# zhenghao2519/Beyond-Fixed-Forms

Measured on AMD Instinct MI355X. Metric: scenes/sec (2D->3D projection+refinement), 200k pts x 300 views, higher is better.
Workload: dtype f64

## Files before the change

### beyond_fixed_forms_amd/_lib.py

```python
from __future__ import annotations

import ctypes
import os
import time
from ctypes import c_double, c_float, c_int32, c_int64, c_void_p

import torch

_HERE = os.path.dirname(os.path.abspath(__file__))
LIB_PATH = os.environ.get("BFF_HIP_LIB") or os.path.join(_HERE, "lib", "libbff_hip.so")
CSRC_DIR = os.path.join(_HERE, "csrc")

_P, _I, _L, _D, _F = c_void_p, c_int32, c_int64, c_double, c_float

SIGNATURES = {
    "bff_rle_to_maskbits": [_P, _P, _P, _P, _I, _L, _I, _P, _P, _P],
    "bff_rle_to_labels": [_P, _P, _P, _P, _I, _L, _I, _P, _P, _P, _P],
    "bff_mask_row_directory": [_P, _P, _P, _I, _I, _I, _P, _P],
    "bff_project_views_lookup": [_P, _L, _L, _P, _P, _I, _P, _I, _I, _I, _P, _I, _I, _D, _P, _P, _P, _P, _P, _I, _P, _P, _P, _P, _P, _L, _L, _P, _P, _P, _P],
    "bff_project_views_cached": [_L, _I, _P, _I, _I, _P, _P, _P, _P, _P, _P, _P, _P, _I, _P, _P, _P, _P, _P, _L, _L, _P, _P, _P, _P],
    "bff_visibility_table": [_P, _L, _L, _P, _P, _I, _P, _I, _I, _I, _I, _I, _D, _P, _P, _P, _P, _L, _P, _I, _P],
    "bff_visibility_sorted": [_P, _P, _P, _L, _L, _I, _I, _I, _P, _P, _P, _P, _P, _P],
    "bff_project_views_runs": [_L, _I, _P, _I, _I, _P, _P, _P, _P, _P, _P, _P, _P, _I, _P, _P, _P, _P, _P, _L, _L, _P, _P, _P, _P],
    "bff_masks2d_count": [_P, _I, _L, _P, _P, _P],
    "bff_masks2d_runs": [_P, _I, _L, _P, _P, _P, _P],
    "bff_project_views": [_P, _L, _L, _P, _P, _I, _P, _P, _I, _I, _D, _P, _P, _P, _I, _P, _P, _P, _P, _P, _L, _L, _P, _P, _P, _P, _P],
    "bff_depth_tile_u16": [_P, _I, _I, _I, _P, _I, _P],
    "bff_project_views_u16": [_P, _L, _L, _P, _P, _I, _P, _I, _I, _I, _P, _I, _I, _D, _P, _P, _P, _I, _P, _P, _P, _P, _P, _L, _L, _P, _P, _P, _P, _P],
    "bff_point_tile_bounds": [_P, _L, _L, _P, _P],
    "bff_count_viewed": [_P, _L, _L, _P, _P, _I, _P, _I, _I, _I, _P, _I, _I, _D, _I, _P, _P, _P],
    "bff_render_depth_u16": [_P, _L, _L, _P, _P, _I, _I, _I, _I, _I, _I, _P, _P, _P, _P],
    "bff_render_splat_depth_u16": [_P, _L, _L, _P, _P, _I, _I, _I, _I, _I, _D, _I, _P, _P, _P, _P],
    "bff_point_labels": [_P, _I, _L, _L, _P, _P, _P],
    "bff_render_labels_u16": [_P, _L, _L, _P, _P, _P, _I, _I, _I, _I, _I, _D, _I, _P, _P, _P, _P, _P],
    "bff_label_runs_count": [_P, _I, _I, _I, _I, _I, _I, _P, _P, _P],
    "bff_label_runs_emit": [_P, _I, _I, _I, _I, _I, _I, _P, _L, _P, _P, _P, _P],
    "bff_render_mesh_depth_u16": [_P, _L, _L, _P, _L, _P, _P, _I, _I, _I, _I, _I, _I, _P, _P, _P],
    "bff_render_mesh_depth_clip_u16": [_P, _L, _L, _P, _L, _P, _P, _I, _I, _I, _I, _I, _D, _I, _P, _P, _P],
# ... 1020 lines not shown
```

### beyond_fixed_forms_amd/csrc/merge.hip

```cpp
#include <hip/hip_ext.h>

#include <cstdlib>

#include "rows.h"

static thread_local hipEvent_t g_merge_start = nullptr, g_merge_stop = nullptr;

namespace bff {

constexpr int kBins = 64;

__device__ __forceinline__ int64_t heavy_signature(uint64_t heavy)
{
    uint32_t key = 0;
#pragma unroll
    for (int s = 0; s < 5; ++s) {
        int b = 63;
        if (heavy) { b = __ffsll((unsigned long long)heavy) - 1; heavy &= heavy - 1; }
        key = (key << 6) | (uint32_t)b;
    }
    return (int64_t)key;
}

__global__ __launch_bounds__(256) void row_stats_kernel(const uint64_t *__restrict__ rows, int64_t nw, int mw,
                                                         int bin_words, int32_t *__restrict__ area,
                                                         int32_t *__restrict__ mean_word,
                                                         uint64_t *__restrict__ cmask, uint32_t *__restrict__ hist,
                                                         int64_t *__restrict__ signature, uint16_t *__restrict__ cpop)
{
    extern __shared__ uint64_t s_cm[];
    __shared__ int part[4];
    __shared__ unsigned long long psum[4];
    __shared__ uint32_t s_hist[kBins];
    const int r = blockIdx.x, tid = threadIdx.x;
    const uint64_t *row = rows + (int64_t)r * nw;
    for (int i = tid; i < mw; i += 256) s_cm[i] = 0;
    if (tid < kBins) s_hist[tid] = 0;
// ... 17 lines not shown
    __syncthreads();
    for (int i = tid; i < mw; i += 256) cmask[(int64_t)r * mw + i] = s_cm[i];
    if (cpop) {
        const int n_chunks = (int)((nw + kCW - 1) / kCW);
        for (int c = tid; c < mw * 64; c += 256) {
            int pc = 0;
            if (c < n_chunks)
#pragma unroll
                for (int k = 0; k < kCW; ++k) { const int64_t w = (int64_t)c * kCW + k; if (w < nw) pc += popc64(row[w]); }
            cpop[(int64_t)r * mw * 64 + c] = (uint16_t)pc;
        }
    }
    const int a_all = part[0] + part[1] + part[2] + part[3];
    if (tid < kBins) {
        hist[(int64_t)r * kBins + tid] = s_hist[tid];
        const uint64_t heavy = __ballot((uint64_t)s_hist[tid] * 100 >= (uint64_t)a_all * 15 && a_all > 0);
        if (tid == 0) signature[r] = heavy_signature(a_all ? heavy : 0);
    }
    if (tid == 0) {
        const int a = part[0] + part[1] + part[2] + part[3];
        const unsigned long long t = psum[0] + psum[1] + psum[2] + psum[3];
        area[r] = a;
        mean_word[r] = a ? (int32_t)(t / (unsigned long long)a) : 0x7fffffff;
    }
}

__global__ __launch_bounds__(256) void row_stats_sparse_kernel(const uint64_t *__restrict__ rows, int n_rows, int64_t nw,
                                                                int mw, int bin_words, int32_t *__restrict__ area,
                                                                int32_t *__restrict__ mean_word,
                                                                const uint64_t *__restrict__ cmask,
                                                                uint32_t *__restrict__ hist, int64_t *__restrict__ signature,
// ... 22 lines not shown
                    const int pc = popc64(v);
                    atomicAdd(&hs[(int)(w / bin_words)], (uint32_t)pc);
                    s += pc;
                    in_chunk += pc;
                    ws += (unsigned long long)pc * (unsigned long long)w;
                }
            }
            if (cpop) cpop[(int64_t)r * mw * 64 + i * 64 + lane] = (uint16_t)in_chunk;
        }
    }
#pragma unroll
    for (int d = 32; d > 0; d >>= 1) { s += __shfl_xor(s, d); ws += __shfl_xor(ws, d); }
    asm volatile("s_waitcnt lgkmcnt(0)" ::: "memory");
    const uint32_t hv = hs[lane];
    hist[(int64_t)r * kBins + lane] = hv;
    const uint64_t heavy = __ballot((uint64_t)hv * 100 >= (uint64_t)s * 15 && s > 0);
    if (lane == 0) {
        signature[r] = heavy_signature(s ? heavy : 0);
        area[r] = s;
        mean_word[r] = s ? (int32_t)(ws / (unsigned long long)s) : 0x7fffffff;
    }
}

__global__ __launch_bounds__(256) void tile_masks_kernel(const uint64_t *__restrict__ cmask,
                                                          const int32_t *__restrict__ order, int n, int mw,
                                                          uint64_t *__restrict__ tmask, const uint32_t *__restrict__ hist,
                                                          uint32_t *__restrict__ hist_sorted, int n_pos,
                                                          const int32_t *__restrict__ area,
                                                          uint32_t *__restrict__ tile_hmax, int32_t *__restrict__ tile_amin,
                                                          const int32_t *__restrict__ label_id,
                                                          int32_t *__restrict__ row_sorted, int32_t *__restrict__ area_sorted,
// ... 817 lines not shown
                             uint16_t *chunk_pop, void *stream)
{
    BFF_REQUIRE(n_rows >= 0 && nw >= 0, "bff_row_stats: bad sizes");
    if (n_rows == 0) return BFF_OK;
    BFF_REQUIRE(rows && area && mean_word && chunk_mask && hist && signature, "bff_row_stats: null pointer");
    const int n_chunks = (int)ceil_div(nw, kCW);
    BFF_LIMIT(n_chunks <= kMaxChunks, "bff_row_stats: more than %d chunks (N > %d points)", kMaxChunks, kMaxChunks * kCW * 64);
    const int mw = (int)ceil_div(n_chunks, 64);
    static_assert(kBins == kWave, "row_stats_sparse_kernel: one histogram bin per lane");
    if (chunk_mask_given) {
        if (chunk_pop) {
            hipError_t e = zero_async(chunk_pop, sizeof(uint16_t) * (size_t)n_rows * mw * 64, as_stream(stream));
            if (e != hipSuccess) return fail((int)e, "bff_row_stats: memset: %s", hipGetErrorString(e));
        }
        row_stats_sparse_kernel<<<(unsigned)ceil_div(n_rows, 4), 256, 0, as_stream(stream)>>>(
            rows, n_rows, nw, mw, (int)ceil_div(nw > 0 ? nw : 1, kBins), area, mean_word, chunk_mask, hist, signature, chunk_pop);
        return launched("bff_row_stats");
    }
    row_stats_kernel<<<n_rows, 256, mw * sizeof(uint64_t), as_stream(stream)>>>(
        rows, nw, mw, (int)ceil_div(nw > 0 ? nw : 1, kBins), area, mean_word, chunk_mask, hist, signature, chunk_pop);
    return launched("bff_row_stats");
}

extern "C" int bff_merge_adjacency(const uint64_t *rows, int32_t n_rows, int64_t nw, const int32_t *order,
                                   const uint64_t *chunk_mask, uint64_t *tile_mask, const uint32_t *hist,
                                   const int32_t *area,
                                   const int32_t *label_id, float iou_thres, uint64_t *adj, int32_t *inter,
                                   void *stream)
{
    BFF_REQUIRE(n_rows >= 0 && nw >= 0, "bff_merge_adjacency: bad sizes");
    if (n_rows == 0) return BFF_OK;
    BFF_REQUIRE(rows && area && label_id && adj, "bff_merge_adjacency: null pointer");
    BFF_REQUIRE((chunk_mask == nullptr) == (tile_mask == nullptr), "bff_merge_adjacency: chunk_mask and tile_mask go together");
    const int nt = (int)ceil_div(n_rows, kT);
    BFF_LIMIT((int64_t)nt * (nt + 1) / 2 < (1ll << 31), "bff_merge_adjacency: too many rows");
// ... 2 lines not shown
    const int mw = (int)ceil_div(n_chunks, 64);
    const bool sparse = chunk_mask && !(0.0f > iou_thres);
    if (sparse) tile_masks_kernel<<<nt, 256, 0, as_stream(stream)>>>(chunk_mask, order, n_rows, mw, tile_mask, nullptr, nullptr, 0, nullptr, nullptr, nullptr,
                                                                     nullptr, nullptr, nullptr, nullptr, nullptr);
    const int aw = nt;
    merge_adjacency_kernel<<<(unsigned)((int64_t)nt * (nt + 1) / 2), 256, 0, as_stream(stream)>>>(
        rows, n_rows, nw, order, sparse ? tile_mask : nullptr, mw, (sparse && !inter) ? hist : nullptr, area, label_id,
        iou_thres, adj, aw, inter, nt);
    return launched("bff_merge_adjacency");
}

extern "C" int32_t bff_merge_uses_chunk_bound(int64_t nw)
{
    static const int forced = [] { const char *e = getenv("BFF_CHUNK_BOUND"); return e ? atoi(e) : -1; }();
    if (forced >= 0) return forced != 0;
    return ceil_div(nw > 0 ? nw : 1, kBins) >= 4 * kCW;
}

struct MergeScratch {
    int64_t n_pos, total, cap2;
    int64_t hist_sorted, tile_hmax, tile_amin;
    int64_t row_sorted, area_sorted, label_sorted;
    int64_t counts, list1, list2;
    int64_t pass2, part2;
    int64_t arrive, partial;
    int64_t words;
};

static MergeScratch merge_scratch_layout(int64_t n)
{
    MergeScratch s;
// ... 117 lines not shown
```

### beyond_fixed_forms_amd/csrc/rows.h

```cpp
#pragma once

#include "common.h"

namespace bff {

constexpr int kT = 64;
constexpr int kKW = 32;
constexpr int kPitch = kT + 1;

__device__ __forceinline__ int uf_find(int32_t *parent, int x)
{
    int p = __hip_atomic_load(parent + x, __ATOMIC_RELAXED, __HIP_MEMORY_SCOPE_AGENT);
    while (p != x) {
        const int g = __hip_atomic_load(parent + p, __ATOMIC_RELAXED, __HIP_MEMORY_SCOPE_AGENT);
        if (g != p) __hip_atomic_store(parent + x, g, __ATOMIC_RELAXED, __HIP_MEMORY_SCOPE_AGENT);
        x = p;
        p = g;
    }
    return x;
}

__device__ __forceinline__ void uf_union(int32_t *parent, int a, int b)
{
    for (;;) {
// ... 20 lines not shown
```

### beyond_fixed_forms_amd/csrc/scene.hip

```cpp
#include "rows.h"

using namespace bff;

namespace {

__global__ void order_keys_kernel(const int64_t *__restrict__ sig, const int32_t *__restrict__ label_id, int n,
                                  int sig_bits, int64_t *__restrict__ keys)
{
    const int i = blockIdx.x * blockDim.x + threadIdx.x;
    if (i < n) keys[i] = ((int64_t)label_id[i] << sig_bits) | sig[i];
}

int bits_for(int n)
{
    int b = 1;
    while ((1 << b) < n && b < 31) ++b;
    return b;
}

}

#define BFF_TRY(call) do { const int rc_ = (call); if (rc_ != BFF_OK) return rc_; } while (0)

extern "C" int32_t bff_scene_header_words(int32_t s1_rows, int32_t cap)
// ... 66 lines not shown
        BFF_TRY(hand_over(ws->events[0], stream, hv));
    }
    const bool cached = lookup && sc->vis_mask && sc->vis_off && sc->vis_pix;
    const bool runs = cached && sc->vis_spix && sc->vis_spt && sc->vis_rowstart && bff_sweep_runs_ok(n) != 0;
    if (lookup && !runs) {
        BFF_REQUIRE(ws->mask_tab && ws->mask_dir, "bff_scene_project: no row directory buffers");
        BFF_TRY(bff_mask_row_directory(sc->run_start, sc->run_end, sc->mask_run_offs, n_rows, sc->height, sc->width,
                                       ws->mask_tab, ws->mask_dir, hv));
    } else if (!lookup) {
        BFF_TRY(bff_rle_to_labels(sc->run_start, sc->run_end, sc->mask_run_offs, sc->view_mask_offs, sc->n_mviews, hw,
                                  sc->word_bits, ws->labels, ws->maskbits, ws->segmap, hv));
    }
    const bool ratio = pr->filter_mode == 2;
    int32_t *const sweep_viewed = (ratio && !viewed_in) ? ws->viewed : nullptr;
    const int32_t *const viewed = ratio ? (viewed_in ? viewed_in : ws->viewed) : nullptr;
    if (runs)
        BFF_TRY(bff_project_views_runs(n, sc->n_frames, sc->depth_index, sc->height, sc->width, sc->vis_mask, sc->vis_spix,
                                       sc->vis_spt, sc->vis_rowstart, sc->run_start, sc->run_end, sc->mask_run_offs,
                                       sc->view_mask_offs, sc->word_bits, sc->frame_mask, sc->frame_rowbase, sc->frame_nmask,
                                       sc->frame_flags, ws->rows, n_rows, nw, ws->chunk_mask, ws->masked, sweep_viewed, hv));
    else if (cached)
        BFF_TRY(bff_project_views_cached(n, sc->n_frames, sc->depth_index, sc->height, sc->width, sc->vis_mask, sc->vis_off,
                                         sc->vis_pix, ws->mask_tab, ws->mask_dir, sc->run_start, sc->run_end,
                                         sc->view_mask_offs, sc->word_bits, sc->frame_mask, sc->frame_rowbase, sc->frame_nmask,
                                         sc->frame_flags, ws->rows, n_rows, nw, ws->chunk_mask, ws->masked, sweep_viewed, hv));
    else if (lookup)
        BFF_TRY(bff_project_views_lookup(sc->xyz, n, sc->n_pad, sc->inv_pose, sc->cam_intr, sc->n_frames,
                                         sc->depth_raw ? sc->depth_raw : (const void *)sc->depth, sc->depth_h, sc->depth_w,
                                         sc->depth_raw ? sc->depth_tiled : -1, sc->depth_index, sc->height, sc->width,
                                         pr->depth_thresh, ws->mask_tab, ws->mask_dir, sc->run_start, sc->run_end,
                                         sc->view_mask_offs, sc->word_bits, sc->frame_mask, sc->frame_rowbase, sc->frame_nmask,
                                         sc->frame_flags, ws->rows, n_rows, nw, ws->chunk_mask, ws->masked, sweep_viewed,
                                         sc->tile_bounds, hv));
    else if (sc->depth_raw)
        BFF_TRY(bff_project_views_u16(sc->xyz, n, sc->n_pad, sc->inv_pose, sc->cam_intr, sc->n_frames, sc->depth_raw,
                                      sc->depth_h, sc->depth_w, sc->depth_tiled, sc->depth_index, sc->height, sc->width, pr->depth_thresh,
// ... 23 lines not shown
        } else {
            BFF_TRY(bff_point_threshold_pairs(ws->masked, viewed, n, pr->filter_fraction,
                                              ws->pair_scratch, reinterpret_cast<float *>(hdr + BFF_HDR_THR),
                                              hdr + BFF_HDR_NUNIQUE, hdr + BFF_HDR_OVERFLOW, stream));
        }
        BFF_TRY(bff_ratio_keep(ws->masked, viewed, n, 0.0f,
                               reinterpret_cast<const float *>(hdr + BFF_HDR_THR), 1, nw, ws->keep, stream));
    } else {
        BFF_TRY(bff_ratio_keep(ws->masked, nullptr, n, 0.0f, nullptr, 0, nw, ws->keep, stream));
    }
    if (fork) {
        hipError_t ee = hipEventRecord(reinterpret_cast<hipEvent_t>(ws->aux_events[1]), as_stream(stream));
        if (ee != hipSuccess) return fail((int)ee, "bff_scene_project: aux stream: %s", hipGetErrorString(ee));
        stream = main_stream;
    }
    uint16_t *cpop = bff_merge_uses_chunk_bound(nw) ? ws->chunk_pop : nullptr;
    BFF_TRY(bff_row_stats(ws->rows, n_rows, nw, ws->area, ws->mean_word, ws->chunk_mask, 1, ws->hist, ws->sig, cpop, stream));
    {
        const int64_t *keys = ws->sig;
        int key_bits = BFF_SIGNATURE_BITS;
        if (sc->n_label_ids > 1) {
            key_bits += bits_for(sc->n_label_ids);
            order_keys_kernel<<<(unsigned)ceil_div(n_rows, 256), 256, 0, st>>>(ws->sig, sc->label_id, n_rows,
                                                                              BFF_SIGNATURE_BITS, ws->sig_keys);
            keys = ws->sig_keys;
        }
        size_t tb = ws->sort_temp_bytes;
        BFF_TRY(bff_argsort_i64(keys, ws->sig_sorted, ws->order, n_rows, key_bits, ws->sort_temp, &tb, stream));
    }
    BFF_TRY(merge_components_streams(ws->rows, n_rows, nw, ws->order, n_rows, ws->chunk_mask, ws->tile_mask, ws->hist,
                                     ws->merge_scratch, ws->area, sc->label_id, pr->iou_thres, ws->parent, 1, nullptr, nullptr,
                                     cpop, stream, hv, ws->events[2], ws->events[3]));
// ... 32 lines not shown
```

### beyond_fixed_forms_amd/csrc/sweep_runs.hip

```cpp
#include <algorithm>
#include <cstdlib>

#include <hip/hip_ext.h>
#include <rocprim/device/device_radix_sort.hpp>

#include "sweep.h"

namespace bff {


__global__ __launch_bounds__(kBlock) void vis_sort_keys_kernel(const uint64_t *__restrict__ mask, const uint32_t *__restrict__ off,
                                                               const uint32_t *__restrict__ pix, int64_t stride, int64_t n_pairs,
                                                               int W, uint32_t hw, uint32_t *__restrict__ keys,
                                                               uint32_t *__restrict__ pts)
{
    const int lane = threadIdx.x & 63;
    const int64_t w = (int64_t)blockIdx.x * (kBlock / kWave) + (threadIdx.x >> 6);
    const int slot = blockIdx.y;
    if (w >= stride) return;
    const uint64_t m = mask[slot * stride + w];
    if (!((m >> lane) & 1)) return;
    const int64_t at = (int64_t)off[slot * stride + w] + __popcll(m & ((1ull << lane) - 1));
    if (at >= n_pairs) return;
    const uint32_t p = pix[at];
// ... 15 lines not shown
    const int64_t t = (int64_t)blockIdx.x * kBlock + threadIdx.x;
    if (t >= (int64_t)n_slots * (H + 1)) return;
    const int s = (int)(t / (H + 1)), y = (int)(t - (int64_t)s * (H + 1));
    int64_t lo = min((int64_t)off[s * stride], n_pairs);
    int64_t hi = s + 1 < n_slots ? min((int64_t)off[(s + 1) * stride], n_pairs) : n_pairs;
    const uint32_t target = (uint32_t)y * (uint32_t)W;
    while (lo < hi) {
        const int64_t mid = lo + ((hi - lo) >> 1);
        if (spix[mid] < target) lo = mid + 1; else hi = mid;
    }
    rowstart[t] = (uint32_t)lo;
}

constexpr int kRunsDeal = 4;

__global__ __launch_bounds__(kBlock) void sweep_runs_fill_kernel(
    int n_frames, const int32_t *__restrict__ depth_index, int H, int W,
    const uint32_t *__restrict__ spix, const uint32_t *__restrict__ spt, const uint32_t *__restrict__ rowstart,
    const int32_t *__restrict__ run_start, const int32_t *__restrict__ run_end, const int32_t *__restrict__ mask_run_offs,
    const int32_t *__restrict__ view_mask_offs, const int32_t *__restrict__ frame_mask,
    const int32_t *__restrict__ frame_rowbase, const int32_t *__restrict__ frame_nmask,
    uint64_t *__restrict__ rows, int64_t nw, int n_chunks, uint64_t *__restrict__ chunk_mask, int mw)
{
    extern __shared__ uint64_t s_row[];
    const int f = blockIdx.x, m = blockIdx.y;
    const int mi = frame_mask[f];
    if (mi < 0 || m >= frame_nmask[f]) return;
    const int tid = threadIdx.x, lane = tid & 63, wave = tid >> 6;
    const int64_t row = (int64_t)frame_rowbase[f] + m;
    for (int i = tid; i < n_chunks * kCW; i += kBlock) s_row[i] = 0;
    __syncthreads();

    const int g = view_mask_offs[mi] + m;
    const int r0 = mask_run_offs[g], r1 = mask_run_offs[g + 1];
    const uint32_t *rs = rowstart + (int64_t)depth_index[f] * (H + 1);
    const int hw = H * W;
    uint32_t *bits = reinterpret_cast<uint32_t *>(s_row);
    for (int rb = r0 + wave * kWave; rb < r1; rb += kBlock) {
        const int r = rb + lane;
        uint32_t lo = 0, cnt = 0;
        if (r < r1) {
            const int start = max(run_start[r], 0), end = min(run_end[r], hw);
            if (start < end) {
                const int y = start / W, ye = (end - 1) / W;
                uint32_t lo1 = rs[y], hi1 = rs[y + 1], lo2 = rs[ye], hi2 = rs[ye + 1];
// ... 48 lines not shown
        for (int h = 0; h < kCW; h += kPPT) {
            uint64_t o = 0;
#pragma unroll
            for (int q = 0; q < kPPT; ++q) o |= v[h + q];
            if (o) {
                any = true;
#pragma unroll
                for (int q = 0; q < kPPT; ++q) {
                    const int64_t w = (int64_t)c * kCW + h + q;
                    if (w < nw) rows[row * nw + w] = v[h + q];
                }
            }
        }
        const uint64_t flags = __ballot(any);
        if (lane == 0 && flags) chunk_mask[row * mw + (c0 >> 6)] |= flags;
    }
}

constexpr int kCountBlock = 1024;
constexpr int kCountBatch = 4;
constexpr int kCountList = 4096;

__global__ __launch_bounds__(kCountBlock) void sweep_runs_count_kernel(const uint64_t *__restrict__ rows, int64_t n_rows, int64_t nw,
                                                                       const uint64_t *__restrict__ chunk_mask, int mw,
                                                                       int64_t n_points, int32_t *__restrict__ masked_count)
{
    __shared__ int s_cnt[kCW * kWave];
    __shared__ int s_list[kCountList];
    __shared__ int s_n;
    const int tid = threadIdx.x, lane = tid & 63, wave = tid >> 6;
    const int c = blockIdx.x;
    static_assert(kCountList == kCountBatch * kCountBlock, "a round lists what one batch of flag loads covers");
    for (int i = tid; i < kCW * kWave; i += kCountBlock) s_cnt[i] = 0;
    int cnt[8] = {};
    const int64_t word = (int64_t)c * kCW + (lane >> 3);
    const int shift = 8 * (lane & 7);
    const uint64_t *flag = chunk_mask + (c >> 6);
    for (int64_t r0 = 0; r0 < n_rows; r0 += kCountList) {
        if (tid == 0) s_n = 0;
        __syncthreads();
        bool set[kCountBatch];
#pragma unroll
        for (int k = 0; k < kCountBatch; ++k) {
            const int64_t r = r0 + k * kCountBlock + tid;
            set[k] = r < n_rows && ((flag[r * mw] >> (c & 63)) & 1);
        }
#pragma unroll
        for (int k = 0; k < kCountBatch; ++k)
            if (set[k]) s_list[atomicAdd(&s_n, 1)] = k * kCountBlock + tid;
        __syncthreads();
        const int n = s_n;
        for (int i0 = wave * kCountBatch; i0 < n; i0 += (kCountBlock / kWave) * kCountBatch) {
            uint64_t v[kCountBatch];
#pragma unroll
            for (int k = 0; k < kCountBatch; ++k)
                v[k] = (i0 + k < n && word < nw) ? rows[(r0 + s_list[i0 + k]) * nw + word] : 0;
#pragma unroll
            for (int k = 0; k < kCountBatch; ++k) {
                const uint32_t b = (uint32_t)(v[k] >> shift) & 0xffu;
#pragma unroll
// ... 7 lines not shown
        if (cnt[q]) atomicAdd(&s_cnt[8 * lane + q], cnt[q]);
    __syncthreads();
    for (int i = tid; i < kCW * kWave; i += kCountBlock) {
        const int64_t n = (int64_t)c * kCW * kWave + i;
        if (n < n_points && s_cnt[i]) masked_count[n] += s_cnt[i];
    }
}

constexpr int kViewedBatch = 4;

__global__ __launch_bounds__(kBlock) void sweep_runs_viewed_kernel(int n_frames, const int32_t *__restrict__ depth_index,
                                                                   const int32_t *__restrict__ frame_flags,
                                                                   const uint64_t *__restrict__ vis_mask, int64_t stride,
                                                                   int64_t nw, int64_t n_points, int32_t *__restrict__ viewed_count)
{
    const int lane = threadIdx.x & 63;
    const int64_t w = (int64_t)blockIdx.x * (kBlock / kWave) + (threadIdx.x >> 6);
    if (w >= nw) return;
    int cnt = 0;
    for (int f0 = 0; f0 < n_frames; f0 += kViewedBatch * kWave) {
        uint64_t m[kViewedBatch];
        int32_t slot[kViewedBatch], flags[kViewedBatch];
#pragma unroll
        for (int k = 0; k < kViewedBatch; ++k) {
            const int f = f0 + k * kWave + lane;
            slot[k] = f < n_frames ? depth_index[f] : 0;
            flags[k] = f < n_frames ? frame_flags[f] : 0;
        }
#pragma unroll
        for (int k = 0; k < kViewedBatch; ++k) m[k] = (flags[k] & 1) ? vis_mask[(int64_t)slot[k] * stride + w] : 0;
#pragma unroll
        for (int k = 0; k < kViewedBatch; ++k) {
            uint64_t live = __ballot(m[k] != 0);
            while (live) {
                const int l = __ffsll((unsigned long long)live) - 1;
                live &= live - 1;
                const uint32_t lo = (uint32_t)__builtin_amdgcn_readlane((int)(uint32_t)m[k], l);
                const uint32_t hi = (uint32_t)__builtin_amdgcn_readlane((int)(uint32_t)(m[k] >> 32), l);
                cnt += (int)(((((uint64_t)hi << 32) | lo) >> lane) & 1);
            }
        }
    }
    const int64_t n = w * kWave + lane;
    if (n < n_points && cnt) viewed_count[n] += cnt;
}

}

using namespace bff;

constexpr int64_t kRunsLdsMax = 64 * 1024;

static int64_t runs_row_bytes(int64_t n_points)
{
    return (int64_t)sizeof(uint64_t) * kCW * ceil_div(ceil_div(n_points, (int64_t)kWave), (int64_t)kCW);
}

extern "C" int32_t bff_sweep_runs_ok(int64_t n_points)
{
    const char *on = getenv("BFF_SWEEP_RUNS"), *cap = getenv("BFF_SWEEP_RUNS_LDS_BYTES");
    if (on && on[0] == '0' && on[1] == 0) return 0;
    int64_t bound = kRunsLdsMax;
    if (cap && *cap) bound = std::min<int64_t>(bound, std::max<int64_t>(0, atoll(cap)));
    return n_points > 0 && runs_row_bytes(n_points) <= bound;
}

extern "C" int bff_project_views_runs(int64_t n_points, int32_t n_frames, const int32_t *depth_index, int32_t height,
                                      int32_t width, const uint64_t *vis_mask, const uint32_t *vis_spix,
                                      const uint32_t *vis_spt, const uint32_t *vis_rowstart, const int32_t *run_start,
                                      const int32_t *run_end, const int32_t *mask_run_offs, const int32_t *view_mask_offs,
                                      int32_t word_bits, const int32_t *frame_mask, const int32_t *frame_rowbase,
                                      const int32_t *frame_nmask, const int32_t *frame_flags, uint64_t *rows, int64_t n_rows,
                                      int64_t nw, uint64_t *chunk_mask, int32_t *masked_count, int32_t *viewed_count,
                                      void *stream)
{
    if (n_points <= 0 || n_frames <= 0) return BFF_OK;
    BFF_REQUIRE(height > 0 && width > 0, "bff_project_views_runs: bad image size");
    BFF_LIMIT((int64_t)height * width < (1ll << 31), "bff_project_views_runs: image larger than 2^31 pixels");
    BFF_REQUIRE(vis_mask && vis_spix && vis_spt && vis_rowstart, "bff_project_views_runs: null table");
    BFF_REQUIRE(word_bits == 32 || word_bits == 64, "bff_project_views_runs: word_bits must be 32 or 64");
    BFF_REQUIRE(depth_index && frame_mask && frame_rowbase && frame_nmask && frame_flags && run_start && run_end &&
                mask_run_offs && view_mask_offs && rows && chunk_mask && n_rows >= 0, "bff_project_views_runs: null pointer");
    BFF_REQUIRE(nw == ceil_div(n_points, 64), "bff_project_views_runs: nw must be ceil(n_points/64)");
    const int64_t row_bytes = runs_row_bytes(n_points);
    BFF_LIMIT(row_bytes <= kRunsLdsMax, "bff_project_views_runs: an instance row exceeds 64 KB of LDS (bff_sweep_runs_ok)");
    hipStream_t st = as_stream(stream);
    const int n_chunks = (int)ceil_div(nw, kCW), mw = (int)ceil_div(n_chunks, 64);
    hipEvent_t ev0, ev1;
    take_sweep_events(&ev0, &ev1);
    const bool count = masked_count != nullptr && n_rows > 0, viewed = viewed_count != nullptr;
    hipExtLaunchKernelGGL(sweep_runs_fill_kernel, dim3((unsigned)n_frames, (unsigned)word_bits), dim3(kBlock),
        (unsigned)row_bytes, st, ev0, (count || viewed) ? nullptr : ev1, 0,
        n_frames, depth_index, height, width, vis_spix, vis_spt, vis_rowstart, run_start, run_end, mask_run_offs,
        view_mask_offs, frame_mask, frame_rowbase, frame_nmask, rows, nw, n_chunks, chunk_mask, mw);
    if (count)
        hipExtLaunchKernelGGL(sweep_runs_count_kernel, dim3((unsigned)n_chunks), dim3(kCountBlock), 0, st,
            nullptr, viewed ? nullptr : ev1, 0, rows, n_rows, nw, chunk_mask, mw, n_points, masked_count);
    if (viewed)
        hipExtLaunchKernelGGL(sweep_runs_viewed_kernel, dim3((unsigned)ceil_div(nw, kBlock / kWave)), dim3(kBlock), 0, st,
            nullptr, ev1, 0, n_frames, depth_index, frame_flags, vis_mask, bff_visibility_words(n_points), nw, n_points,
            viewed_count);
    return launched("bff_project_views_runs");
}

extern "C" int bff_visibility_sorted_bytes(int32_t n_slots, int32_t height, int64_t n_pixels, int64_t *bytes)
{
    BFF_REQUIRE(n_slots >= 0 && height >= 0 && n_pixels >= 0 && bytes, "bff_visibility_sorted_bytes: bad arguments");
    bytes[0] = (int64_t)sizeof(uint32_t) * n_pixels;
    bytes[1] = (int64_t)sizeof(uint32_t) * n_pixels;
    bytes[2] = (int64_t)sizeof(uint32_t) * n_slots * ((int64_t)height + 1);
    return BFF_OK;
}

extern "C" int bff_visibility_sorted(const uint64_t *vis_mask, const uint32_t *vis_off, const uint32_t *vis_pix,
                                     int64_t n_pixels, int64_t n_points, int32_t n_slots, int32_t height, int32_t width,
                                     uint32_t *vis_spix, uint32_t *vis_spt, uint32_t *vis_rowstart, void *temp,
                                     size_t *temp_bytes, void *stream)
// ... 38 lines not shown
```

### include/bff_hip.h

```cpp
#ifndef BFF_HIP_H
#define BFF_HIP_H

#include <stddef.h>
#include <stdint.h>

#ifdef __cplusplus
extern "C" {
#endif

#define BFF_OK 0
#define BFF_E_ARG (-1)
#define BFF_E_LIMIT (-2)

#define BFF_ABI_VERSION 16

int bff_abi_version(void);
const char *bff_last_error(void);
const char *bff_arch(void);

int bff_host_component_csr(const int32_t *comp, const uint8_t *has_self_loop, int32_t n, int32_t min_members,
                           int32_t *offs, int32_t *members, int32_t *sizes, int32_t *n_void);

int bff_rle_to_maskbits(const int32_t *run_start, const int32_t *run_end, const int32_t *mask_run_offs,
                        const int32_t *view_mask_offs, int32_t n_views, int64_t n_pixels, int32_t word_bits,
// ... 246 lines not shown
                             int32_t *masked_count, int32_t *viewed_count, void *stream);

int bff_visibility_sorted(const uint64_t *vis_mask, const uint32_t *vis_off, const uint32_t *vis_pix, int64_t n_pixels,
                          int64_t n_points, int32_t n_slots, int32_t height, int32_t width, uint32_t *vis_spix,
                          uint32_t *vis_spt, uint32_t *vis_rowstart, void *temp, size_t *temp_bytes, void *stream);
int bff_visibility_sorted_bytes(int32_t n_slots, int32_t height, int64_t n_pixels, int64_t *bytes);

int32_t bff_sweep_runs_ok(int64_t n_points);
int bff_project_views_runs(int64_t n_points, int32_t n_frames, const int32_t *depth_index, int32_t height, int32_t width,
                           const uint64_t *vis_mask, const uint32_t *vis_spix, const uint32_t *vis_spt,
                           const uint32_t *vis_rowstart, const int32_t *run_start, const int32_t *run_end,
                           const int32_t *mask_run_offs, const int32_t *view_mask_offs, int32_t word_bits,
                           const int32_t *frame_mask, const int32_t *frame_rowbase, const int32_t *frame_nmask,
                           const int32_t *frame_flags, uint64_t *rows, int64_t n_rows, int64_t nw, uint64_t *chunk_mask,
                           int32_t *masked_count, int32_t *viewed_count, void *stream);

typedef struct bff_scene {
    int64_t n_points, n_pad, nw;
    const double *xyz;
    const double *tile_bounds;
    const double *inv_pose;
    double cam_intr[9];
    const float *depth;
    const void *depth_raw;
    const int32_t *depth_index, *frame_mask, *frame_rowbase, *frame_nmask, *frame_flags;
    const int32_t *run_start, *run_end, *mask_run_offs, *view_mask_offs;
    const void *conf;
    const int32_t *label_id;
    const int32_t *unsort;
    const int32_t *perm;
// ... 151 lines not shown
```

Before: 1542.

## Fuse row statistics into runs sweep fill kernel and transpose chunk flags

Computes per-row area, mean word, histogram, heavy-bin signature and chunk popcounts inside the runs fill kernel while the row is still in LDS, so the separate row_stats pass over all rows is skipped on the runs path. The fill kernel also writes a transposed chunk-flag table into the mask_dir scratch, giving the count kernel contiguous flag reads. The viewed kernel is restructured so one block covers one word, with its waves splitting the frames and reducing through shared memory. In exchange the fill kernel gains LDS atomics and register pressure, and mask_dir is reused as scratch, which depends on the height/alignment check.

New measurement: 1508. -2.2%, worse.

```diff
diff --git a/beyond_fixed_forms_amd/_lib.py b/beyond_fixed_forms_amd/_lib.py
--- a/beyond_fixed_forms_amd/_lib.py
+++ b/beyond_fixed_forms_amd/_lib.py
@@ -22,6 +22,7 @@
     "bff_visibility_table": [_P, _L, _L, _P, _P, _I, _P, _I, _I, _I, _I, _I, _D, _P, _P, _P, _P, _L, _P, _I, _P],
     "bff_visibility_sorted": [_P, _P, _P, _L, _L, _I, _I, _I, _P, _P, _P, _P, _P, _P],
     "bff_project_views_runs": [_L, _I, _P, _I, _I, _P, _P, _P, _P, _P, _P, _P, _P, _I, _P, _P, _P, _P, _P, _L, _L, _P, _P, _P, _P],
+    "bff_project_views_runs_stats": [_L, _I, _P, _I, _I, _P, _P, _P, _P, _P, _P, _P, _P, _I, _P, _P, _P, _P, _P, _L, _L, _P, _P, _P] + [_P] * 7,
     "bff_masks2d_count": [_P, _I, _L, _P, _P, _P],
     "bff_masks2d_runs": [_P, _I, _L, _P, _P, _P, _P],
     "bff_project_views": [_P, _L, _L, _P, _P, _I, _P, _P, _I, _I, _D, _P, _P, _P, _I, _P, _P, _P, _P, _P, _L, _L, _P, _P, _P, _P, _P],
diff --git a/beyond_fixed_forms_amd/csrc/merge.hip b/beyond_fixed_forms_amd/csrc/merge.hip
--- a/beyond_fixed_forms_amd/csrc/merge.hip
+++ b/beyond_fixed_forms_amd/csrc/merge.hip
@@ -8,19 +8,6 @@
 
 namespace bff {
 
-constexpr int kBins = 64;
-
-__device__ __forceinline__ int64_t heavy_signature(uint64_t heavy)
-{
-    uint32_t key = 0;
-#pragma unroll
-    for (int s = 0; s < 5; ++s) {
-        int b = 63;
-        if (heavy) { b = __ffsll((unsigned long long)heavy) - 1; heavy &= heavy - 1; }
-        key = (key << 6) | (uint32_t)b;
-    }
-    return (int64_t)key;
-}
 
 __global__ __launch_bounds__(256) void row_stats_kernel(const uint64_t *__restrict__ rows, int64_t nw, int mw,
                                                          int bin_words, int32_t *__restrict__ area,
@@ -68,7 +55,7 @@
     const int a_all = part[0] + part[1] + part[2] + part[3];
     if (tid < kBins) {
         hist[(int64_t)r * kBins + tid] = s_hist[tid];
-        const uint64_t heavy = __ballot((uint64_t)s_hist[tid] * 100 >= (uint64_t)a_all * 15 && a_all > 0);
+        const uint64_t heavy = __ballot(heavy_bin(s_hist[tid], a_all));
         if (tid == 0) signature[r] = heavy_signature(a_all ? heavy : 0);
     }
     if (tid == 0) {
@@ -121,7 +108,7 @@
     asm volatile("s_waitcnt lgkmcnt(0)" ::: "memory");
     const uint32_t hv = hs[lane];
     hist[(int64_t)r * kBins + lane] = hv;
-    const uint64_t heavy = __ballot((uint64_t)hv * 100 >= (uint64_t)s * 15 && s > 0);
+    const uint64_t heavy = __ballot(heavy_bin(hv, s));
     if (lane == 0) {
         signature[r] = heavy_signature(s ? heavy : 0);
         area[r] = s;
@@ -969,11 +956,11 @@
             if (e != hipSuccess) return fail((int)e, "bff_row_stats: memset: %s", hipGetErrorString(e));
         }
         row_stats_sparse_kernel<<<(unsigned)ceil_div(n_rows, 4), 256, 0, as_stream(stream)>>>(
-            rows, n_rows, nw, mw, (int)ceil_div(nw > 0 ? nw : 1, kBins), area, mean_word, chunk_mask, hist, signature, chunk_pop);
+            rows, n_rows, nw, mw, stats_bin_words(nw), area, mean_word, chunk_mask, hist, signature, chunk_pop);
         return launched("bff_row_stats");
     }
     row_stats_kernel<<<n_rows, 256, mw * sizeof(uint64_t), as_stream(stream)>>>(
-        rows, nw, mw, (int)ceil_div(nw > 0 ? nw : 1, kBins), area, mean_word, chunk_mask, hist, signature, chunk_pop);
+        rows, nw, mw, stats_bin_words(nw), area, mean_word, chunk_mask, hist, signature, chunk_pop);
     return launched("bff_row_stats");
 }
 
@@ -1006,7 +993,7 @@
 {
     static const int forced = [] { const char *e = getenv("BFF_CHUNK_BOUND"); return e ? atoi(e) : -1; }();
     if (forced >= 0) return forced != 0;
-    return ceil_div(nw > 0 ? nw : 1, kBins) >= 4 * kCW;
+    return stats_bin_words(nw) >= 4 * kCW;
 }
 
 struct MergeScratch {
diff --git a/beyond_fixed_forms_amd/csrc/rows.h b/beyond_fixed_forms_amd/csrc/rows.h
--- a/beyond_fixed_forms_amd/csrc/rows.h
+++ b/beyond_fixed_forms_amd/csrc/rows.h
@@ -7,6 +7,27 @@
 constexpr int kT = 64;
 constexpr int kKW = 32;
 constexpr int kPitch = kT + 1;
+
+constexpr int kBins = 64;
+
+inline int stats_bin_words(int64_t nw) { return (int)ceil_div(nw > 0 ? nw : (int64_t)1, (int64_t)kBins); }
+
+__device__ __forceinline__ bool heavy_bin(uint32_t bin_count, int area)
+{
+    return area > 0 && (uint64_t)bin_count * 100 >= (uint64_t)area * 15;
+}
+
+__device__ __forceinline__ int64_t heavy_signature(uint64_t heavy)
+{
+    uint32_t key = 0;
+#pragma unroll
+    for (int s = 0; s < 5; ++s) {
+        int b = 63;
+        if (heavy) { b = __ffsll((unsigned long long)heavy) - 1; heavy &= heavy - 1; }
+        key = (key << 6) | (uint32_t)b;
+    }
+    return (int64_t)key;
+}
 
 __device__ __forceinline__ int uf_find(int32_t *parent, int x)
 {
diff --git a/beyond_fixed_forms_amd/csrc/scene.hip b/beyond_fixed_forms_amd/csrc/scene.hip
--- a/beyond_fixed_forms_amd/csrc/scene.hip
+++ b/beyond_fixed_forms_amd/csrc/scene.hip
@@ -104,12 +104,17 @@
     const bool ratio = pr->filter_mode == 2;
     int32_t *const sweep_viewed = (ratio && !viewed_in) ? ws->viewed : nullptr;
     const int32_t *const viewed = ratio ? (viewed_in ? viewed_in : ws->viewed) : nullptr;
-    if (runs)
-        BFF_TRY(bff_project_views_runs(n, sc->n_frames, sc->depth_index, sc->height, sc->width, sc->vis_mask, sc->vis_spix,
-                                       sc->vis_spt, sc->vis_rowstart, sc->run_start, sc->run_end, sc->mask_run_offs,
-                                       sc->view_mask_offs, sc->word_bits, sc->frame_mask, sc->frame_rowbase, sc->frame_nmask,
-                                       sc->frame_flags, ws->rows, n_rows, nw, ws->chunk_mask, ws->masked, sweep_viewed, hv));
-    else if (cached)
+    uint16_t *cpop = bff_merge_uses_chunk_bound(nw) ? ws->chunk_pop : nullptr;
+    if (runs) {
+        const bool fits = ws->mask_dir && sc->height >= 2 * mw && reinterpret_cast<uintptr_t>(ws->mask_dir) % sizeof(uint64_t) == 0;
+        uint64_t *flags_t = fits ? reinterpret_cast<uint64_t *>(ws->mask_dir) : nullptr;
+        BFF_TRY(bff_project_views_runs_stats(n, sc->n_frames, sc->depth_index, sc->height, sc->width, sc->vis_mask,
+                                             sc->vis_spix, sc->vis_spt, sc->vis_rowstart, sc->run_start, sc->run_end,
+                                             sc->mask_run_offs, sc->view_mask_offs, sc->word_bits, sc->frame_mask,
+                                             sc->frame_rowbase, sc->frame_nmask, sc->frame_flags, ws->rows, n_rows, nw,
+                                             ws->chunk_mask, ws->masked, sweep_viewed, ws->area, ws->mean_word, ws->hist,
+                                             ws->sig, cpop, flags_t, hv));
+    } else if (cached)
         BFF_TRY(bff_project_views_cached(n, sc->n_frames, sc->depth_index, sc->height, sc->width, sc->vis_mask, sc->vis_off,
                                          sc->vis_pix, ws->mask_tab, ws->mask_dir, sc->run_start, sc->run_end,
                                          sc->view_mask_offs, sc->word_bits, sc->frame_mask, sc->frame_rowbase, sc->frame_nmask,
@@ -163,8 +168,8 @@
         if (ee != hipSuccess) return fail((int)ee, "bff_scene_project: aux stream: %s", hipGetErrorString(ee));
         stream = main_stream;
     }
-    uint16_t *cpop = bff_merge_uses_chunk_bound(nw) ? ws->chunk_pop : nullptr;
-    BFF_TRY(bff_row_stats(ws->rows, n_rows, nw, ws->area, ws->mean_word, ws->chunk_mask, 1, ws->hist, ws->sig, cpop, stream));
+    if (!runs)
+        BFF_TRY(bff_row_stats(ws->rows, n_rows, nw, ws->area, ws->mean_word, ws->chunk_mask, 1, ws->hist, ws->sig, cpop, stream));
     {
         const int64_t *keys = ws->sig;
         int key_bits = BFF_SIGNATURE_BITS;
diff --git a/beyond_fixed_forms_amd/csrc/sweep_runs.hip b/beyond_fixed_forms_amd/csrc/sweep_runs.hip
--- a/beyond_fixed_forms_amd/csrc/sweep_runs.hip
+++ b/beyond_fixed_forms_amd/csrc/sweep_runs.hip
@@ -4,6 +4,7 @@
 #include <hip/hip_ext.h>
 #include <rocprim/device/device_radix_sort.hpp>
 
+#include "rows.h"
 #include "sweep.h"
 
 namespace bff {
@@ -53,21 +54,29 @@
 
 constexpr int kRunsDeal = 4;
 
+template <bool kStats>
 __global__ __launch_bounds__(kBlock) void sweep_runs_fill_kernel(
     int n_frames, const int32_t *__restrict__ depth_index, int H, int W,
     const uint32_t *__restrict__ spix, const uint32_t *__restrict__ spt, const uint32_t *__restrict__ rowstart,
     const int32_t *__restrict__ run_start, const int32_t *__restrict__ run_end, const int32_t *__restrict__ mask_run_offs,
     const int32_t *__restrict__ view_mask_offs, const int32_t *__restrict__ frame_mask,
     const int32_t *__restrict__ frame_rowbase, const int32_t *__restrict__ frame_nmask,
-    uint64_t *__restrict__ rows, int64_t nw, int n_chunks, uint64_t *__restrict__ chunk_mask, int mw)
+    uint64_t *__restrict__ rows, int64_t nw, int n_chunks, uint64_t *__restrict__ chunk_mask, int mw,
+    int64_t n_rows, int bin_words, uint64_t bin_magic, int32_t *__restrict__ area, int32_t *__restrict__ mean_word, uint32_t *__restrict__ hist,
+    int64_t *__restrict__ signature, uint16_t *__restrict__ chunk_pop, uint64_t *__restrict__ flags_t)
 {
     extern __shared__ uint64_t s_row[];
+    __shared__ uint32_t s_hist[kBins];
+    __shared__ uint32_t s_area;
+    __shared__ unsigned long long s_wsum;
     const int f = blockIdx.x, m = blockIdx.y;
     const int mi = frame_mask[f];
     if (mi < 0 || m >= frame_nmask[f]) return;
     const int tid = threadIdx.x, lane = tid & 63, wave = tid >> 6;
     const int64_t row = (int64_t)frame_rowbase[f] + m;
     for (int i = tid; i < n_chunks * kCW; i += kBlock) s_row[i] = 0;
+    if (kStats && tid < kBins) s_hist[tid] = 0;
+    if (kStats && tid == 0) { s_area = 0; s_wsum = 0; }
     __syncthreads();
 
     const int g = view_mask_offs[mi] + m;
@@ -146,6 +155,56 @@
         }
         const uint64_t flags = __ballot(any);
         if (lane == 0 && flags) chunk_mask[row * mw + (c0 >> 6)] |= flags;
+        if constexpr (kStats) {
+            if (lane == 0 && flags_t) flags_t[(int64_t)(c0 >> 6) * n_rows + row] = flags;
+            if (any) {
+                const int w0 = c * kCW;
+                int pc[kCW], in_chunk = 0, by_q = 0;
+#pragma unroll
+                for (int q = 0; q < kCW; ++q) {
+                    pc[q] = w0 + q < nw ? popc64(v[q]) : 0;
+                    in_chunk += pc[q];
+                    by_q += q * pc[q];
+                }
+                const int bin0 = (int)(((uint64_t)(uint32_t)w0 * bin_magic) >> 32);
+                const int left = (bin0 + 1) * bin_words - w0;
+                if (left >= kCW) {
+                    atomicAdd(&s_hist[bin0], (uint32_t)in_chunk);
+                } else {
+                    int bin = bin0, l = left;
+                    uint32_t acc = 0;
+#pragma unroll
+                    for (int q = 0; q < kCW; ++q) {
+                        acc += (uint32_t)pc[q];
+                        if (--l == 0) {
+                            if (acc) atomicAdd(&s_hist[bin], acc);
+                            acc = 0;
+                            ++bin;
+                            l = bin_words;
+                        }
+                    }
+                    if (acc) atomicAdd(&s_hist[bin], acc);
+                }
+                atomicAdd(&s_area, (uint32_t)in_chunk);
+                atomicAdd(&s_wsum, (unsigned long long)(uint32_t)(w0 * in_chunk + by_q));
+                if (chunk_pop) chunk_pop[row * mw * 64 + c] = (uint16_t)in_chunk;
+            }
+        }
+    }
+    if constexpr (kStats) {
+        __syncthreads();
+        static_assert(kBins == kWave, "one histogram bin per lane of the first wave");
+        if (wave == 0) {
+            const uint32_t a = s_area, hv = s_hist[lane];
+            const unsigned long long t = s_wsum;
+            hist[row * kBins + lane] = hv;
+            const uint64_t heavy = __ballot(heavy_bin(hv, (int)a));
+            if (lane == 0) {
+                signature[row] = heavy_signature(a ? heavy : 0);
+                area[row] = (int32_t)a;
+                mean_word[row] = !a ? 0x7fffffff : (t >> 32) ? (int32_t)(t / a) : (int32_t)((uint32_t)t / a);
+            }
+        }
     }
 }
 
@@ -155,7 +214,8 @@
 
 __global__ __launch_bounds__(kCountBlock) void sweep_runs_count_kernel(const uint64_t *__restrict__ rows, int64_t n_rows, int64_t nw,
                                                                        const uint64_t *__restrict__ chunk_mask, int mw,
-                                                                       int64_t n_points, int32_t *__restrict__ masked_count)
+                                                                       int64_t n_points, int32_t *__restrict__ masked_count,
+                                                                       const uint64_t *__restrict__ flags_t)
 {
     __shared__ int s_cnt[kCW * kWave];
     __shared__ int s_list[kCountList];
@@ -168,6 +228,7 @@
     const int64_t word = (int64_t)c * kCW + (lane >> 3);
     const int shift = 8 * (lane & 7);
     const uint64_t *flag = chunk_mask + (c >> 6);
+    const uint64_t *flag_t = flags_t ? flags_t + (int64_t)(c >> 6) * n_rows : nullptr;
     for (int64_t r0 = 0; r0 < n_rows; r0 += kCountList) {
         if (tid == 0) s_n = 0;
         __syncthreads();
@@ -175,7 +236,7 @@
 #pragma unroll
         for (int k = 0; k < kCountBatch; ++k) {
             const int64_t r = r0 + k * kCountBlock + tid;
-            set[k] = r < n_rows && ((flag[r * mw] >> (c & 63)) & 1);
+            set[k] = r < n_rows && (((flag_t ? flag_t[r] : flag[r * mw]) >> (c & 63)) & 1);
         }
 #pragma unroll
         for (int k = 0; k < kCountBatch; ++k)
@@ -213,16 +274,16 @@
                                                                    const uint64_t *__restrict__ vis_mask, int64_t stride,
                                                                    int64_t nw, int64_t n_points, int32_t *__restrict__ viewed_count)
 {
-    const int lane = threadIdx.x & 63;
-    const int64_t w = (int64_t)blockIdx.x * (kBlock / kWave) + (threadIdx.x >> 6);
-    if (w >= nw) return;
+    __shared__ int s_cnt[kBlock / kWave - 1][kWave];
+    const int lane = threadIdx.x & 63, wave = threadIdx.x >> 6;
+    const int64_t w = blockIdx.x;
     int cnt = 0;
-    for (int f0 = 0; f0 < n_frames; f0 += kViewedBatch * kWave) {
+    for (int f0 = wave * kWave; f0 < n_frames; f0 += kViewedBatch * kBlock) {
         uint64_t m[kViewedBatch];
         int32_t slot[kViewedBatch], flags[kViewedBatch];
 #pragma unroll
         for (int k = 0; k < kViewedBatch; ++k) {
-            const int f = f0 + k * kWave + lane;
+            const int f = f0 + k * kBlock + lane;
             slot[k] = f < n_frames ? depth_index[f] : 0;
             flags[k] = f < n_frames ? frame_flags[f] : 0;
         }
@@ -240,6 +301,11 @@
             }
         }
     }
+    if (wave) s_cnt[wave - 1][lane] = cnt;
+    __syncthreads();
+    if (wave) return;
+#pragma unroll
+    for (int k = 0; k < kBlock / kWave - 1; ++k) cnt += s_cnt[k][lane];
     const int64_t n = w * kWave + lane;
     if (n < n_points && cnt) viewed_count[n] += cnt;
 }
@@ -262,6 +328,68 @@
     int64_t bound = kRunsLdsMax;
     if (cap && *cap) bound = std::min<int64_t>(bound, std::max<int64_t>(0, atoll(cap)));
     return n_points > 0 && runs_row_bytes(n_points) <= bound;
+}
+
+struct RunsStats {
+    int32_t *area, *mean_word;
+    uint32_t *hist;
+    int64_t *signature;
+    uint16_t *chunk_pop;
+    uint64_t *flags_t;
+};
+
+static int project_views_runs(const char *who, int64_t n_points, int32_t n_frames, const int32_t *depth_index, int32_t height,
+                              int32_t width, const uint64_t *vis_mask, const uint32_t *vis_spix, const uint32_t *vis_spt,
+                              const uint32_t *vis_rowstart, const int32_t *run_start, const int32_t *run_end,
+                              const int32_t *mask_run_offs, const int32_t *view_mask_offs, int32_t word_bits,
+                              const int32_t *frame_mask, const int32_t *frame_rowbase, const int32_t *frame_nmask,
+                              const int32_t *frame_flags, uint64_t *rows, int64_t n_rows, int64_t nw, uint64_t *chunk_mask,
+                              int32_t *masked_count, int32_t *viewed_count, const RunsStats *stats, void *stream)
+{
+    if (n_points <= 0 || n_frames <= 0) return BFF_OK;
+    BFF_REQUIRE(height > 0 && width > 0, "%s: bad image size", who);
+    BFF_LIMIT((int64_t)height * width < (1ll << 31), "%s: image larger than 2^31 pixels", who);
+    BFF_REQUIRE(vis_mask && vis_spix && vis_spt && vis_rowstart, "%s: null table", who);
+    BFF_REQUIRE(word_bits == 32 || word_bits == 64, "%s: word_bits must be 32 or 64", who);
+    BFF_REQUIRE(depth_index && frame_mask && frame_rowbase && frame_nmask && frame_flags && run_start && run_end &&
+                mask_run_offs && view_mask_offs && rows && chunk_mask && n_rows >= 0, "%s: null pointer", who);
+    BFF_REQUIRE(!stats || (stats->area && stats->mean_word && stats->hist && stats->signature),
+                "%s: null statistics pointer", who);
+    BFF_REQUIRE(nw == ceil_div(n_points, 64), "%s: nw must be ceil(n_points/64)", who);
+    const int64_t row_bytes = runs_row_bytes(n_points);
+    BFF_LIMIT(row_bytes <= kRunsLdsMax, "%s: an instance row exceeds 64 KB of LDS (bff_sweep_runs_ok)", who);
+    hipStream_t st = as_stream(stream);
+    const int n_chunks = (int)ceil_div(nw, kCW), mw = (int)ceil_div(n_chunks, 64);
+    if (stats && stats->chunk_pop && n_rows > 0) {
+        hipError_t e = zero_async(stats->chunk_pop, sizeof(uint16_t) * (size_t)n_rows * mw * 64, st);
+        if (e != hipSuccess) return fail((int)e, "%s: memset: %s", who, hipGetErrorString(e));
+    }
+    hipEvent_t ev0, ev1;
+    take_sweep_events(&ev0, &ev1);
+    const bool count = masked_count != nullptr && n_rows > 0, viewed = viewed_count != nullptr;
+    const dim3 grid((unsigned)n_frames, (unsigned)word_bits);
+    hipEvent_t fill_stop = (count || viewed) ? nullptr : ev1;
+    if (stats)
+        hipExtLaunchKernelGGL(sweep_runs_fill_kernel<true>, grid, dim3(kBlock), (unsigned)row_bytes, st, ev0, fill_stop, 0,
+            n_frames, depth_index, height, width, vis_spix, vis_spt, vis_rowstart, run_start, run_end, mask_run_offs,
+            view_mask_offs, frame_mask, frame_rowbase, frame_nmask, rows, nw, n_chunks, chunk_mask, mw, n_rows,
+            stats_bin_words(nw), ((1ull << 32) + stats_bin_words(nw) - 1) / stats_bin_words(nw), stats->area, stats->mean_word, stats->hist, stats->signature, stats->chunk_pop,
+            stats->flags_t);
+    else
+        hipExtLaunchKernelGGL(sweep_runs_fill_kernel<false>, grid, dim3(kBlock), (unsigned)row_bytes, st, ev0, fill_stop, 0,
+            n_frames, depth_index, height, width, vis_spix, vis_spt, vis_rowstart, run_start, run_end, mask_run_offs,
+            view_mask_offs, frame_mask, frame_rowbase, frame_nmask, rows, nw, n_chunks, chunk_mask, mw, n_rows, 0,
+            (uint64_t)0, (int32_t *)nullptr, (int32_t *)nullptr, (uint32_t *)nullptr, (int64_t *)nullptr, (uint16_t *)nullptr,
+            (uint64_t *)nullptr);
+    if (count)
+        hipExtLaunchKernelGGL(sweep_runs_count_kernel, dim3((unsigned)n_chunks), dim3(kCountBlock), 0, st,
+            nullptr, viewed ? nullptr : ev1, 0, rows, n_rows, nw, chunk_mask, mw, n_points, masked_count,
+            stats ? (const uint64_t *)stats->flags_t : (const uint64_t *)nullptr);
+    if (viewed)
+        hipExtLaunchKernelGGL(sweep_runs_viewed_kernel, dim3((unsigned)nw), dim3(kBlock), 0, st,
+            nullptr, ev1, 0, n_frames, depth_index, frame_flags, vis_mask, bff_visibility_words(n_points), nw, n_points,
+            viewed_count);
+    return launched(who);
 }
 
 extern "C" int bff_project_views_runs(int64_t n_points, int32_t n_frames, const int32_t *depth_index, int32_t height,
@@ -273,33 +401,28 @@
                                       int64_t nw, uint64_t *chunk_mask, int32_t *masked_count, int32_t *viewed_count,
                                       void *stream)
 {
-    if (n_points <= 0 || n_frames <= 0) return BFF_OK;
-    BFF_REQUIRE(height > 0 && width > 0, "bff_project_views_runs: bad image size");
-    BFF_LIMIT((int64_t)height * width < (1ll << 31), "bff_project_views_runs: image larger than 2^31 pixels");
-    BFF_REQUIRE(vis_mask && vis_spix && vis_spt && vis_rowstart, "bff_project_views_runs: null table");
-    BFF_REQUIRE(word_bits == 32 || word_bits == 64, "bff_project_views_runs: word_bits must be 32 or 64");
-    BFF_REQUIRE(depth_index && frame_mask && frame_rowbase && frame_nmask && frame_flags && run_start && run_end &&
-                mask_run_offs && view_mask_offs && rows && chunk_mask && n_rows >= 0, "bff_project_views_runs: null pointer");
-    BFF_REQUIRE(nw == ceil_div(n_points, 64), "bff_project_views_runs: nw must be ceil(n_points/64)");
-    const int64_t row_bytes = runs_row_bytes(n_points);
-    BFF_LIMIT(row_bytes <= kRunsLdsMax, "bff_project_views_runs: an instance row exceeds 64 KB of LDS (bff_sweep_runs_ok)");
-    hipStream_t st = as_stream(stream);
-    const int n_chunks = (int)ceil_div(nw, kCW), mw = (int)ceil_div(n_chunks, 64);
-    hipEvent_t ev0, ev1;
-    take_sweep_events(&ev0, &ev1);
-    const bool count = masked_count != nullptr && n_rows > 0, viewed = viewed_count != nullptr;
-    hipExtLaunchKernelGGL(sweep_runs_fill_kernel, dim3((unsigned)n_frames, (unsigned)word_bits), dim3(kBlock),
-        (unsigned)row_bytes, st, ev0, (count || viewed) ? nullptr : ev1, 0,
-        n_frames, depth_index, height, width, vis_spix, vis_spt, vis_rowstart, run_start, run_end, mask_run_offs,
-        view_mask_offs, frame_mask, frame_rowbase, frame_nmask, rows, nw, n_chunks, chunk_mask, mw);
-    if (count)
-        hipExtLaunchKernelGGL(sweep_runs_count_kernel, dim3((unsigned)n_chunks), dim3(kCountBlock), 0, st,
-            nullptr, viewed ? nullptr : ev1, 0, rows, n_rows, nw, chunk_mask, mw, n_points, masked_count);
-    if (viewed)
-        hipExtLaunchKernelGGL(sweep_runs_viewed_kernel, dim3((unsigned)ceil_div(nw, kBlock / kWave)), dim3(kBlock), 0, st,
-            nullptr, ev1, 0, n_frames, depth_index, frame_flags, vis_mask, bff_visibility_words(n_points), nw, n_points,
-            viewed_count);
-    return launched("bff_project_views_runs");
+    return project_views_runs("bff_project_views_runs", n_points, n_frames, depth_index, height, width, vis_mask, vis_spix,
+                              vis_spt, vis_rowstart, run_start, run_end, mask_run_offs, view_mask_offs, word_bits, frame_mask,
+                              frame_rowbase, frame_nmask, frame_flags, rows, n_rows, nw, chunk_mask, masked_count,
+                              viewed_count, nullptr, stream);
+}
+
+extern "C" int bff_project_views_runs_stats(int64_t n_points, int32_t n_frames, const int32_t *depth_index, int32_t height,
+                                            int32_t width, const uint64_t *vis_mask, const uint32_t *vis_spix,
+                                            const uint32_t *vis_spt, const uint32_t *vis_rowstart, const int32_t *run_start,
+                                            const int32_t *run_end, const int32_t *mask_run_offs,
+                                            const int32_t *view_mask_offs, int32_t word_bits, const int32_t *frame_mask,
+                                            const int32_t *frame_rowbase, const int32_t *frame_nmask,
+                                            const int32_t *frame_flags, uint64_t *rows, int64_t n_rows, int64_t nw,
+                                            uint64_t *chunk_mask, int32_t *masked_count, int32_t *viewed_count, int32_t *area,
+                                            int32_t *mean_word, uint32_t *hist, int64_t *signature, uint16_t *chunk_pop,
+                                            uint64_t *flags_t, void *stream)
+{
+    const RunsStats stats = {area, mean_word, hist, signature, chunk_pop, flags_t};
+    return project_views_runs("bff_project_views_runs_stats", n_points, n_frames, depth_index, height, width, vis_mask,
+                              vis_spix, vis_spt, vis_rowstart, run_start, run_end, mask_run_offs, view_mask_offs, word_bits,
+                              frame_mask, frame_rowbase, frame_nmask, frame_flags, rows, n_rows, nw, chunk_mask, masked_count,
+                              viewed_count, &stats, stream);
 }
 
 extern "C" int bff_visibility_sorted_bytes(int32_t n_slots, int32_t height, int64_t n_pixels, int64_t *bytes)
diff --git a/include/bff_hip.h b/include/bff_hip.h
--- a/include/bff_hip.h
+++ b/include/bff_hip.h
@@ -284,6 +284,14 @@
                            const int32_t *frame_mask, const int32_t *frame_rowbase, const int32_t *frame_nmask,
                            const int32_t *frame_flags, uint64_t *rows, int64_t n_rows, int64_t nw, uint64_t *chunk_mask,
                            int32_t *masked_count, int32_t *viewed_count, void *stream);
+int bff_project_views_runs_stats(int64_t n_points, int32_t n_frames, const int32_t *depth_index, int32_t height,
+                                 int32_t width, const uint64_t *vis_mask, const uint32_t *vis_spix, const uint32_t *vis_spt,
+                                 const uint32_t *vis_rowstart, const int32_t *run_start, const int32_t *run_end,
+                                 const int32_t *mask_run_offs, const int32_t *view_mask_offs, int32_t word_bits,
+                                 const int32_t *frame_mask, const int32_t *frame_rowbase, const int32_t *frame_nmask,
+                                 const int32_t *frame_flags, uint64_t *rows, int64_t n_rows, int64_t nw, uint64_t *chunk_mask,
+                                 int32_t *masked_count, int32_t *viewed_count, int32_t *area, int32_t *mean_word,
+                                 uint32_t *hist, int64_t *signature, uint16_t *chunk_pop, uint64_t *flags_t, void *stream);
 
 typedef struct bff_scene {
     int64_t n_points, n_pad, nw;
```
